# NVIDIA/nv-wavenet

Measured on AMD Instinct MI355X. Metric: samples/sec (all GPUs) in real time (every utterance >= 24 kHz) and max real-time batch @24kHz, R64/S256/A256 20L fp16, higher is better.
Workload: dtype f16; 1 GPU; C3: R=64 S=256 A=256 L=20 maxDilation=512 fp16, autoregressive generation at steady state (each step = samples 640..895 of every utterance: all dilated taps live, all rings wrapped; the steps re-run that sample range -- same launch, same memory traffic -- so from the second step on the rings hold the previous step's values: a timing workload, not one long utterance); batch_per_gpu=12288, global_batch=12288, parallelism=batch-sharded x1, final RCCL all_gather

## Files before the change

### nv_wavenet_amd/csrc/wn_experiments.hpp

```cpp
#pragma once

#ifndef WN_PFMAX
#define WN_PFMAX 12
#endif
#ifndef WN_PFMAX_FEAT
#define WN_PFMAX_FEAT 12
#endif
#ifndef WN_HEADREGS
#define WN_HEADREGS 128
#endif
#ifndef WN_HEADREGS2
#define WN_HEADREGS2 128
#endif
#ifndef WN_HEADREGS3
#define WN_HEADREGS3 0
#endif
#ifndef WN_COND_VALU
#define WN_COND_VALU 1
#endif
#ifndef WN_LDS_RING_MAXD
#define WN_LDS_RING_MAXD 512
#endif
#ifndef WN_SOFTMAX_2PASS
#define WN_SOFTMAX_2PASS 0
#endif
#ifndef WN_CHAIN_HOIST_FROM
#define WN_CHAIN_HOIST_FROM 4
#endif
#ifndef WN_WG4_FROM
#define WN_WG4_FROM 3
#endif
#ifndef WN_HEADREGS4
#define WN_HEADREGS4 0
#endif
#ifndef WN_ZS_B_REGS
#define WN_ZS_B_REGS 4096
#endif
#ifndef WN_ZA_B_REGS
#define WN_ZA_B_REGS 128
#endif
#ifndef WN_TAKE_G
#define WN_TAKE_G 1
#endif
#ifndef WN_REQ_AT
#define WN_REQ_AT 6
#endif
#ifndef WN_REQ_AT_FEAT
#define WN_REQ_AT_FEAT 6
#endif
#ifndef WN_UP_PHASES
#define WN_UP_PHASES(F16) 1
#endif
#ifndef WN_UP_COLS
#define WN_UP_COLS(F16) (WN_UP_PHASES(F16) > 1 ? 2 : 4)
#endif
#ifndef WN_UP_WAVES
#define WN_UP_WAVES(F16) (WN_UP_PHASES(F16) > 1 ? 8 : 4)
#endif
#ifndef WN_UP_ATTR
#define WN_UP_ATTR
#endif
#ifndef WN_W_AUX
#define WN_W_AUX 0
#endif
#ifndef WN_RING_LD_AUX
#define WN_RING_LD_AUX 2
#endif
#ifndef WN_RING_ST_AUX
#define WN_RING_ST_AUX 2
#endif
#ifndef WN_COND_AUX
#define WN_COND_AUX 2
#endif
#ifndef WN_RAW_AUX
#define WN_RAW_AUX 0
#endif
#ifndef WN_FEAT_AUX
#define WN_FEAT_AUX 0
#endif
```

### nv_wavenet_amd/csrc/wn_kernels.hpp

```cpp
#pragma once

#include <hip/hip_runtime.h>
#include <utility>
#include <stdint.h>

#include <type_traits>

#include "wn_experiments.hpp"

namespace wn {

#define WN_DEV __device__ __forceinline__

typedef _Float16 half8 __attribute__((ext_vector_type(8)));
typedef _Float16 half4 __attribute__((ext_vector_type(4)));
typedef float floatx4 __attribute__((ext_vector_type(4)));
typedef unsigned int uintx4 __attribute__((ext_vector_type(4)));
typedef unsigned int uintx2 __attribute__((ext_vector_type(2)));

template <bool F16> struct Prec;
template <> struct Prec<true> {
    using elem = _Float16;
    using frag = half8;
    using quad = half4;
    static constexpr int EPL = 8;
    static constexpr int TPF = 2;
};
template <> struct Prec<false> {
    using elem = float;
    using frag = floatx4;
    using quad = floatx4;
    static constexpr int EPL = 4;
    static constexpr int TPF = 1;
};

constexpr int kMaxLayers = 128;

constexpr int pick_pf(int fl, int pfmax) {
    int best = 1;
    for (int d = 1; d <= pfmax && d <= fl; d++)
        if (fl % d == 0) best = d;
    return best;
}
constexpr int align16(int x) { return (x + 15) & ~15; }

constexpr int kCondChannelsMax = 80;
template <bool F16> constexpr int feat_kfc() { return (kCondChannelsMax + 16 * Prec<F16>::TPF - 1) / (16 * Prec<F16>::TPF); }

template <bool F16, int R, int S, int A, int BT, int KFC = 0>
struct Cfg {
    using P = Prec<F16>;
    static constexpr int TPF = P::TPF, EPL = P::EPL;
    static constexpr int RT = R / 16, ST = S / 16, AT = A / 16;
    static constexpr int NW = RT >= 4 ? 4 : RT;
    static_assert(R % (16 * TPF) == 0 && S % (16 * TPF) == 0 && A % (16 * TPF) == 0, "R,S,A vs MFMA K step");
    static_assert(RT % NW == 0 && ST % NW == 0 && AT % NW == 0, "tiles must split evenly over the waves");
    static constexpr int THREADS = NW * 64;
    static constexpr int HTW = RT / NW, STW = ST / NW, ATW = AT / NW;
    static constexpr int KF_R = RT / TPF, KF_S = ST / TPF, KF_A = AT / TPF;
    static constexpr int FW_GATE = 2 * HTW * KF_R, FW_RES = HTW * KF_R, FW_SKIP = STW * KF_R, FW_COND = 2 * HTW * KFC;
    static constexpr int O_PREV = 0, O_CUR = FW_GATE, O_RES = 2 * FW_GATE, O_SKIP = O_RES + FW_RES, O_COND = O_SKIP + FW_SKIP;
    static constexpr int FLW = O_COND + FW_COND;
    __host__ __device__ static constexpr size_t streamPos(int l, int i, int L) {
        return i < O_CUR    ? (size_t)((l == 0 ? L : l) - 1) * FLW + FW_GATE + FW_COND + FW_RES + (i - O_PREV)
               : i < O_RES  ? (l == 0 ? (size_t)(i - O_CUR) : (size_t)l * FLW - FW_SKIP + (i - O_CUR))
               : i < O_SKIP ? (size_t)l * FLW + FW_GATE + FW_COND + (i - O_RES)
               : i < O_COND ? (l == L - 1 ? (size_t)L * FLW - FW_SKIP + (i - O_SKIP)
                                          : (size_t)(l + 1) * FLW - FW_SKIP + FW_GATE + (i - O_SKIP))
                            : (size_t)((l == 0 ? L : l) - 1) * FLW + FW_GATE + (i - O_COND);
    }
    static constexpr int P_CUR0 = FLW, P_CUR = FLW - FW_SKIP, P_SKIP = P_CUR + FW_GATE, P_COND = FLW + FW_GATE,
                         P_RES = P_COND + FW_COND, P_PREV = P_RES + FW_RES;
    static constexpr int FW_ZS = ATW * KF_S, FW_ZA = ATW * KF_A;
    static constexpr int FHW = FW_ZS + FW_ZA;
    static constexpr int PF = pick_pf(FLW, KFC > 0 ? WN_PFMAX_FEAT : WN_PFMAX);
    static_assert(FLW % PF == 0 && PF <= FW_ZS, "prefetch ring must divide the layer stream");
    static constexpr int HR = !F16 ? 0
                              : BT == 1 ? (FW_ZA * 4 <= WN_HEADREGS ? FW_ZA : 0)
                              : BT == 2 ? (FW_ZA * 4 <= WN_HEADREGS2 ? FW_ZA : 0)
                              : BT == 3 ? (FW_ZA * 4 <= WN_HEADREGS3 ? FW_ZA : 0)
                                        : (FW_ZA * 4 <= WN_HEADREGS4 ? FW_ZA : 0);
    static constexpr int HS = FHW - HR;
    static constexpr bool HEADRES = HS == 0;
    static constexpr int PAD1 = (PF - FW_ZS % PF) % PF, PAD2 = (PF - FW_ZA % PF) % PF;
    static constexpr int O_ZS = 0, O_ZA = FW_ZS + PAD1;
    static constexpr int FHWP = O_ZA + FW_ZA + PAD2;
    static constexpr int HSP = HS == 0 ? 0 : (HS == FW_ZS ? FW_ZS + PAD1 : FHWP);
    static_assert(HS == 0 || HS == FW_ZS || HS == FHW, "the streamed part of the head is nothing, zs, or all of it");
    __host__ __device__ static constexpr int headFrag(int q) { return q < FW_ZS ? q : q + PAD1; }
    static constexpr int FRAG_ELEMS = 64 * EPL;
    static constexpr int BIAS_L = 3 * R + S;
    static constexpr int COND_FR = 2 * HTW / TPF;
    static constexpr int LPU = 4 * NW;
    static constexpr int RPL = A / LPU;
    static_assert(RPL % 4 == 0, "A too small for the softmax lane split");
    static constexpr int XBUF = BT * KF_R * 1024;
    static constexpr int HBUF = XBUF;
    static constexpr int SKBUF = BT * KF_S * 1024;
    static constexpr int ZSBUF = BT * KF_A * 1024;
    static constexpr int LROW = A + 4;
    static constexpr int LGT = (BT >= 4 && WN_SOFTMAX_2PASS) ? 2 : BT;
    static_assert(BT % LGT == 0, "the softmax passes take whole groups of tiles");
    static constexpr int LGBUF = LGT * 16 * LROW * 4;
    static constexpr int YBUF = align16(BT * 16 * 4);
    static constexpr int XPBUF = XBUF;
    static constexpr int XPW = (KF_R + NW - 1) / NW;
    static constexpr bool ALIAS_LG = ZSBUF + LGBUF > 100 * 1024 || BT >= 3;
    static constexpr bool ZA_B_FROM_LDS = KF_A * BT * 4 > WN_ZA_B_REGS;
    static constexpr int HEADIMG = ALIAS_LG ? (ZSBUF > LGBUF ? ZSBUF : LGBUF) : ZSBUF + LGBUF;
    static constexpr bool OVERLAY = XBUF + HBUF + XPBUF <= (ALIAS_LG ? HEADIMG : LGBUF);
    static constexpr int OFF_SK = OVERLAY ? 0 : XBUF + HBUF, OFF_ZS = OFF_SK + SKBUF;
    static constexpr int OFF_LG = ALIAS_LG ? OFF_ZS : OFF_ZS + ZSBUF;
    static constexpr int OFF_Y = OFF_ZS + HEADIMG;
    static constexpr int OFF_X = OVERLAY ? OFF_LG : 0, OFF_H = OFF_X + XBUF, OFF_XP = OVERLAY ? OFF_H + HBUF : OFF_Y + YBUF;
    static constexpr int OFF_BIAS = OVERLAY ? OFF_Y + YBUF : OFF_XP + XPBUF;
    static constexpr int LDS_FIXED = XBUF + HBUF + SKBUF + HEADIMG + YBUF + XPBUF;
    static constexpr int BIAS_LN = 3 * R;
    __host__ __device__ static constexpr int biasFloats(int L, bool dump) { return (dump ? L * BIAS_L : L * BIAS_LN + S) + 2 * A; }
    __host__ __device__ static constexpr size_t ldsBytes(int L, int embTables, bool dump = true) {
        return (size_t)LDS_FIXED + (size_t)biasFloats(L, dump) * sizeof(float) + (size_t)embTables * A * R * sizeof(typename P::elem);
    }
    static constexpr int RING_SLOT = BT * KF_R * 1024;
    static constexpr int RING_INPLACE = OVERLAY ? 3 : 0;
    static_assert(XBUF == RING_SLOT && HBUF == RING_SLOT && XPBUF == RING_SLOT, "a vacated exchange image is one ring slot");
    static_assert(OFF_BIAS + RING_INPLACE * RING_SLOT == LDS_FIXED, "the in-place slots are what LDS_FIXED counts behind the tables");
    __host__ __device__ static constexpr int ringSlotOffset(int slot, int tailBase) { return tailBase + (slot - RING_INPLACE) * RING_SLOT; }
    __host__ __device__ static constexpr int ringTailSlots(int slots) { return slots > RING_INPLACE ? slots - RING_INPLACE : 0; }
    __host__ __device__ static constexpr int ldsRingSlots(int L, int maxDilation, int D) {
        int n = 0, d = 1;
        for (int l = 0; l < L; l++) {
            if (d <= D) n += d;
            d <<= 1;
            if (d > maxDilation) d = 1;
        }
        return n;
    }
    __host__ __device__ static size_t headOffsetFrags(int L) { return (size_t)L * FLW; }
    __host__ __device__ static size_t waveStreamFrags(int L) { return (size_t)L * FLW + FHWP; }
};

struct Dil {
    int d, off, lds;
};
WN_DEV Dil dil_first() { return Dil{1, 0, 0}; }
WN_DEV Dil dil_next(Dil s, int maxDilation, bool wrapToFirst, int ldsD = 0) {
    Dil n;
    n.off = s.off + s.d;
    n.lds = s.lds + (s.d <= ldsD ? s.d : 0);
    n.d = s.d << 1;
    if (n.d > maxDilation) n.d = 1;
    if (wrapToFirst) n = dil_first();
    return n;
}

struct Params {
    const void* wblob;
    const float* bias;
    const void* embPrev;
    const void* embCur;
    const void* cond;
    const void* condRaw;
    int condRawKind;
    const void* feat;
    const unsigned* gate;
    const float* sel;
    void* ring;
    int maxDilation;
    int* yInPrev;
    int* yInCur;
    int* yOut;
    float* xtOut;
    float* skipOut;
// ... 140 lines not shown
    if constexpr (PIN) return __builtin_bit_cast(FRAG, agpr_pin(__builtin_bit_cast(floatx4, f)));
    else return f;
}

template <bool F16, int PF, bool PIN = F16> struct WStream {
    typename Prec<F16>::frag buf[PF];
};

template <bool F16, int PF, int WRAP, bool PIN>
WN_DEV typename Prec<F16>::frag take(WStream<F16, PF, PIN>& ws, int idx, const char* base, const char* wrapBase,
                                     unsigned laneOff, int rtWrapAt = 0x7fffffff, long rtWrapDelta = 0) {
    using frag = typename Prec<F16>::frag;
    frag a = agpr_operand<F16 && PIN>(ws.buf[idx % PF]);
    int nidx = idx + PF;
    const char* src = (WRAP > 0 && nidx >= WRAP) ? wrapBase + (size_t)(nidx - WRAP) * 1024 : base + (size_t)nidx * 1024;
    if (nidx >= rtWrapAt) src += rtWrapDelta;
    ws.buf[idx % PF] = *(const frag*)(src + laneOff);
    __builtin_amdgcn_sched_barrier(0);
    return a;
}

template <bool F16, int PF, int WRAP, int BT, int MT, int KF, bool PIN>
WN_DEV void gemm(WStream<F16, PF, PIN>& ws, int pos0, const char* cur, const char* next, unsigned laneOff,
                 floatx4 (&acc)[BT][MT], const typename Prec<F16>::frag (&b)[BT][KF], int rtWrapAt = 0x7fffffff,
                 long rtWrapDelta = 0) {
    constexpr int G = MT >= 4 ? 4 : MT;
#pragma unroll
    for (int mg = 0; mg < MT / G; mg++) {
#pragma unroll
        for (int kf = 0; kf < KF; kf++) {
#pragma unroll
            for (int mi = 0; mi < G; mi++) {
                const int mt = mg * G + mi;
                auto a = take<F16, PF, WRAP>(ws, pos0 + (mg * KF + kf) * G + mi, cur, next, laneOff, rtWrapAt, rtWrapDelta);
#pragma unroll
                for (int bt = 0; bt < BT; bt++) acc[bt][mt] = mma(a, b[bt][kf], acc[bt][mt]);
            }
        }
    }
}

template <bool F16, int PF, int WRAP, int BT, int MT, int KF, bool PIN>
WN_DEV void gemm_ldsb(WStream<F16, PF, PIN>& ws, int pos0, const char* cur, const char* next, unsigned laneOff,
                      floatx4 (&acc)[BT][MT], const char* bimg, int lane) {
    using frag = typename Prec<F16>::frag;
    constexpr int G = MT >= 4 ? 4 : MT;
#pragma unroll
    for (int mg = 0; mg < MT / G; mg++) {
#pragma unroll
        for (int kf = 0; kf < KF; kf++) {
            frag b[BT];
#pragma unroll
            for (int bt = 0; bt < BT; bt++) b[bt] = *(const frag*)(bimg + (((bt * KF + kf) * 64 + lane) << 4));
#pragma unroll
            for (int mi = 0; mi < G; mi++) {
                const int mt = mg * G + mi;
                auto a = take<F16, PF, WRAP>(ws, pos0 + (mg * KF + kf) * G + mi, cur, next, laneOff);
#pragma unroll
                for (int bt = 0; bt < BT; bt++) acc[bt][mt] = mma(a, b[bt], acc[bt][mt]);
            }
        }
    }
}

typedef __amdgpu_buffer_rsrc_t rsrc_t;
__host__ __device__ constexpr int take_g(int g, int pf) {
    int t = g < WN_TAKE_G ? g : WN_TAKE_G;
    t = t < pf ? t : pf;
    while (g % t) t--;
    return t;
}
WN_DEV rsrc_t make_rsrc(const void* p) { return __builtin_amdgcn_make_buffer_rsrc((void*)p, 0, -1, 0x00020000); }
template <typename FRAG, int AUX = 0> WN_DEV FRAG buf_load(rsrc_t rs, unsigned voff, unsigned soff) {
    return __builtin_bit_cast(FRAG, __builtin_amdgcn_raw_buffer_load_b128(rs, voff, soff, AUX));
}
template <typename FRAG, int AUX = 0> WN_DEV void buf_store(rsrc_t rs, unsigned voff, unsigned soff, FRAG v) {
    __builtin_amdgcn_raw_buffer_store_b128(__builtin_bit_cast(uintx4, v), rs, voff, soff, AUX);
}
template <bool F16, int PF, bool PIN, int G>
WN_DEV void take_group(WStream<F16, PF, PIN>& ws, int idx, typename Prec<F16>::frag (&a)[G]) {
#pragma unroll
    for (int i = G - 1; i >= 0; i--) a[i] = agpr_operand<F16 && PIN>(ws.buf[(idx + i) % PF]);
}
template <bool F16, int PF, int WRAP, bool PIN, int G>
WN_DEV void refill_group(WStream<F16, PF, PIN>& ws, rsrc_t rs, int idx, int basePos, int wrapPos, unsigned laneOff) {
    using frag = typename Prec<F16>::frag;
#pragma unroll
    for (int i = 0; i < G; i++) {
        const int nidx = idx + i + PF;
        const bool wr = WRAP > 0 && nidx >= WRAP;
        const int rel = wr ? nidx - WRAP : nidx;
        const int pos = (wr ? wrapPos : basePos) + (rel & ~3);
        ws.buf[(idx + i) % PF] = buf_load<frag, WN_W_AUX>(rs, laneOff + (unsigned)(rel & 3) * 1024u, (unsigned)pos * 1024u);
    }
    __builtin_amdgcn_sched_barrier(0);
}
template <bool F16, int PF, int WRAP, int BT, int MT, int KF, bool PIN>
WN_DEV void gemm_b(WStream<F16, PF, PIN>& ws, rsrc_t rs, int pos0, int basePos, int wrapPos, unsigned laneOff,
                   floatx4 (&acc)[BT][MT], const typename Prec<F16>::frag (&b)[BT][KF]) {
    constexpr int G = MT >= 4 ? 4 : MT;
#pragma unroll
    for (int mg = 0; mg < MT / G; mg++) {
#pragma unroll
        for (int kf = 0; kf < KF; kf++) {
            constexpr int TG = take_g(G, PF);
#pragma unroll
            for (int m0 = 0; m0 < G; m0 += TG) {
                typename Prec<F16>::frag a[TG];
                const int idx = pos0 + (mg * KF + kf) * G + m0;
                take_group<F16, PF, PIN, TG>(ws, idx, a);
                constexpr bool EARLY = PF > TG;
                if (EARLY && !(mg == 0 && kf == 0 && m0 == 0)) refill_group<F16, PF, WRAP, PIN, TG>(ws, rs, idx - TG, basePos, wrapPos, laneOff);
#pragma unroll
                for (int mi = 0; mi < TG; mi++)
#pragma unroll
                    for (int bt = 0; bt < BT; bt++)
                        acc[bt][mg * G + m0 + mi] = mma(a[mi], b[bt][kf], acc[bt][mg * G + m0 + mi]);
                if (!EARLY || (mg == MT / G - 1 && kf == KF - 1 && m0 + TG >= G)) refill_group<F16, PF, WRAP, PIN, TG>(ws, rs, idx, basePos, wrapPos, laneOff);
            }
        }
    }
}
template <bool F16, int PF, int WRAP, int BT, int MT, int KF, bool PIN>
WN_DEV void gemm_ldsb_b(WStream<F16, PF, PIN>& ws, rsrc_t rs, int pos0, int basePos, int wrapPos, unsigned laneOff,
                        floatx4 (&acc)[BT][MT], const char* bimg, int lane) {
    using frag = typename Prec<F16>::frag;
    constexpr int G = MT >= 4 ? 4 : MT;
#pragma unroll
    for (int mg = 0; mg < MT / G; mg++) {
#pragma unroll
        for (int kf = 0; kf < KF; kf++) {
            frag b[BT];
#pragma unroll
            for (int bt = 0; bt < BT; bt++) b[bt] = *(const frag*)(bimg + (((bt * KF + kf) * 64 + lane) << 4));
            constexpr int TG = take_g(G, PF);
#pragma unroll
            for (int m0 = 0; m0 < G; m0 += TG) {
                frag a[TG];
                take_group<F16, PF, PIN, TG>(ws, pos0 + (mg * KF + kf) * G + m0, a);
#pragma unroll
                for (int mi = 0; mi < TG; mi++)
#pragma unroll
                    for (int bt = 0; bt < BT; bt++) acc[bt][mg * G + m0 + mi] = mma(a[mi], b[bt], acc[bt][mg * G + m0 + mi]);
                refill_group<F16, PF, WRAP, PIN, TG>(ws, rs, pos0 + (mg * KF + kf) * G + m0, basePos, wrapPos, laneOff);
            }
        }
    }
}
template <bool F16, int PF, int WRAP, bool PIN, int N>
WN_DEV void skip_frags(WStream<F16, PF, PIN>& ws, rsrc_t rs, int idx, int basePos, int wrapPos, unsigned laneOff) {
    if constexpr (N > 0) {
        typename Prec<F16>::frag a[N];
        take_group<F16, PF, PIN, N>(ws, idx, a);
        refill_group<F16, PF, WRAP, PIN, N>(ws, rs, idx, basePos, wrapPos, laneOff);
    }
}

template <bool F16, int BT, int MT, int KF>
WN_DEV void gemm_direct(const char* src, unsigned laneOff, floatx4 (&acc)[BT][MT], const typename Prec<F16>::frag (&b)[BT][KF]) {
    using frag = typename Prec<F16>::frag;
    constexpr int G = MT >= 4 ? 4 : MT;
#pragma unroll
    for (int mg = 0; mg < MT / G; mg++)
#pragma unroll
        for (int kf = 0; kf < KF; kf++)
#pragma unroll
            for (int mi = 0; mi < G; mi++) {
                const frag a = *(const frag*)(src + (size_t)((mg * KF + kf) * G + mi) * 1024 + laneOff);
#pragma unroll
                for (int bt = 0; bt < BT; bt++) acc[bt][mg * G + mi] = mma(a, b[bt][kf], acc[bt][mg * G + mi]);
            }
}

template <bool F16, int BT, int MT, int KF, int NFR>
WN_DEV void gemm_res(const typename Prec<F16>::frag (&wres)[NFR], int pos0, floatx4 (&acc)[BT][MT],
                     const typename Prec<F16>::frag (&b)[BT][KF]) {
    constexpr int G = MT >= 4 ? 4 : MT;
#pragma unroll
    for (int mg = 0; mg < MT / G; mg++)
#pragma unroll
        for (int kf = 0; kf < KF; kf++)
#pragma unroll
            for (int mi = 0; mi < G; mi++)
#pragma unroll
                for (int bt = 0; bt < BT; bt++)
                    acc[bt][mg * G + mi] = mma(agpr_operand<F16>(wres[pos0 + (mg * KF + kf) * G + mi]), b[bt][kf], acc[bt][mg * G + mi]);
}

template <int CTRL> WN_DEV float dpp_f(float v) {
    return __int_as_float(__builtin_amdgcn_update_dpp(0, __float_as_int(v), CTRL, 0xf, 0xf, false));
}
template <int CTRL> WN_DEV int dpp_i(int v) { return __builtin_amdgcn_update_dpp(0, v, CTRL, 0xf, 0xf, false); }
constexpr int DPP_XOR1 = 0xB1, DPP_XOR2 = 0x4E;
constexpr int DPP_HALF_MIRROR = 0x141, DPP_MIRROR = 0x140;
template <int LPU, typename F> WN_DEV float group_reduce_f(float v, F op) {
    static_assert(LPU == 4 || LPU == 8 || LPU == 16, "softmax lanes per utterance");
    v = op(v, dpp_f<DPP_XOR1>(v));
    v = op(v, dpp_f<DPP_XOR2>(v));
    if (LPU >= 8) v = op(v, dpp_f<DPP_HALF_MIRROR>(v));
    if (LPU >= 16) v = op(v, dpp_f<DPP_MIRROR>(v));
    return v;
}
template <int LPU> WN_DEV int group_min_i(int v) {
    int o = dpp_i<DPP_XOR1>(v); v = o < v ? o : v;
    o = dpp_i<DPP_XOR2>(v); v = o < v ? o : v;
    if (LPU >= 8) { o = dpp_i<DPP_HALF_MIRROR>(v); v = o < v ? o : v; }
    if (LPU >= 16) { o = dpp_i<DPP_MIRROR>(v); v = o < v ? o : v; }
    return v;
}

template <int A, int LPU, int RPL>
WN_DEV int softmax_pick(const float* lrow, int sq, int lane, float sel, float (&e)[RPL], float& total) {
    (void)lane;
#pragma unroll
    for (int i = 0; i < RPL / 4; i++) {
        floatx4 v = *(const floatx4*)(lrow + i * 4);
#pragma unroll
        for (int r = 0; r < 4; r++) e[i * 4 + r] = v[r];
    }
    float m = e[0];
#pragma unroll
    for (int i = 1; i < RPL; i++) m = __builtin_fmaxf(m, e[i]);
    m = group_reduce_f<LPU>(m, [](float a, float b) { return __builtin_fmaxf(a, b); });
    float lsum = 0.f;
    {
        constexpr float kLog2e = 1.44269504088896340736f;
        const float mneg = -m * kLog2e;
#pragma unroll
        for (int i = 0; i < RPL; i++) {
            e[i] = __builtin_amdgcn_exp2f(__builtin_fmaf(e[i], kLog2e, mneg));
            lsum += e[i];
        }
    }
    float incl = lsum;
    {
        float up = dpp_f<0x111>(incl);
        if (sq >= 1) incl += up;
        up = dpp_f<0x112>(incl);
// ... 333 lines not shown
    for (int tt = 0; tt < P::TPF; tt++)
#pragma unroll
        for (int e = 0; e < P::EPL; e++)
            selA[tt][e] = (elem)(((e >> 2) == tt && g * 4 + (e & 3) == j) ? 1.0f : 0.0f);
    floatx4 acc[BT][2 * HTW];
    {
        frag xp[BT][KF_R];
#pragma unroll
        for (int bt = 0; bt < BT; bt++) {
            lds_get_frags<F16, KF_R>(tap_image(p.dil[0], p.initSample) + bt * KF_R * 1024, lane, xp[bt]);
#pragma unroll
            for (int i = 0; i < HTW; i++) {
                acc[bt][2 * i] = *(const floatx4*)(biasLds + (w + NW * i) * 16 + g * 4);
                acc[bt][2 * i + 1] = *(const floatx4*)(biasLds + (w + NW * i + RT) * 16 + g * 4);
            }
        }
        if constexpr (FEAT) {
            load_feat(p.initSample, cfNext);
#pragma unroll
            for (int bt = 0; bt < BT; bt++)
#pragma unroll
                for (int k = 0; k < KFC; k++) cfCur[bt][k] = agpr_operand<F16>(cfNext[bt][k]);
            gemm_direct<F16, BT, 2 * HTW, KFC>(wbase + C::streamPos(0, C::O_COND, L) * 1024, laneOff, acc, cfCur);
            load_feat(p.initSample + 1, cfNext);
#pragma unroll
            for (int bt = 0; bt < BT; bt++)
#pragma unroll
                for (int k = 0; k < KFC; k++) asm volatile("" ::"v"(cfNext[bt][k]));
        } else {
#pragma unroll
            for (int bt = 0; bt < BT; bt++)
#pragma unroll
                for (int k = 0; k < C::COND_FR; k++) cond_add<F16>(&acc[bt][k * P::TPF], cond_frag<F16, RAW>(cdA[bt], k), selA);
        }
        gemm_direct<F16, BT, 2 * HTW, KF_R>(wbase + C::streamPos(0, C::O_PREV, L) * 1024, laneOff, acc, xp);
    }
    const int tEnd = p.initSample + p.count;
    for (int t = p.initSample; t < tEnd; t++) {
        const bool dumpNow = DUMP && p.dump && (t == tEnd - 1);

        float selv[BT];
        if (!p.useRng) {
#pragma unroll
            for (int bt = 0; bt < BT; bt++) {
                int sb = (tile0 + bt) * 16 + su;
                sb = sb < p.batch ? sb : p.batch - 1;
                selv[bt] = p.sel[(size_t)t * p.maxBatch + sb];
            }
        }

        WN_TMARK(11)
        floatx4 x[BT][HTW];
#pragma unroll
        for (int bt = 0; bt < BT; bt++) {
#pragma unroll
            for (int i = 0; i < HTW; i++) {
                const int tile = w + NW * i;
                floatx4 ec = quad_to_f32(*(const quad*)(embCur + (size_t)yCur[bt] * R + tile * 16 + g * 4));
                floatx4 v = ep[bt][i] + ec;
                if (p.tanhEmbed) {
#pragma unroll
                    for (int r = 0; r < 4; r++) v[r] = tanh_t<F16>(v[r]);
                }
                x[bt][i] = v;
                lds_put_tile<F16>(xbuf + bt * KF_R * 1024, tile, lane, v);
            }
#pragma unroll
            for (int i = 0; i < HTW; i++)
                ep[bt][i] = quad_to_f32(*(const quad*)(embPrev + (size_t)yCur[bt] * R + (w + NW * i) * 16 + g * 4));
        }
        wg_barrier();
        WN_TMARK(0)

        floatx4 skip[BT][STW];
#pragma unroll
        for (int bt = 0; bt < BT; bt++)
#pragma unroll
            for (int i = 0; i < STW; i++) skip[bt][i] = floatx4{0.f, 0.f, 0.f, 0.f};

        frag hb[BT][KF_R];
        frag xb[BT][KF_R];
#pragma unroll
        for (int bt = 0; bt < BT; bt++) lds_get_frags<F16, KF_R>(xbuf + bt * KF_R * 1024, lane, xb[bt]);
        auto layer = [&](auto withSkip, const int l, const Dil dl, const Dil dN, const Dil dl2, frag (&xpC)[BT][XPW],
                         frag (&cdC)[BT][CR], const frag (&xpN)[BT][XPW], const frag (&cdN)[BT][CR]) {
            constexpr bool SKIP = decltype(withSkip)::value;
            constexpr int PB = SKIP ? 0 : FLW;
            const int wl = SKIP ? (l - 1) * FLW : 0;
            const float* bl = biasLds + l * BLS;
            const int lN = l + 1 < L ? l + 1 : 0;
            const float* blN = biasLds + lN * BLS;
            const int d = dl.d;

            WN_TMARK(1)
            gemm_b<F16, PF, 0, BT, 2 * HTW, KF_R>(ws, rsW, SKIP ? C::P_CUR : C::P_CUR0 - PB, wl, 0, laneOff, acc, xb);
            const bool ringInLds = d <= ldsD;
            frag xkeep[BT][XPW];
            if (!ringInLds) {
                const unsigned rp = (unsigned)(dl.off + (t & (d - 1))) * (unsigned)(KF_R * 1024);
#pragma unroll
                for (int k = 0; k < KF_R; k++)
                    if (k % NW == w) {
#pragma unroll
                        for (int bt = 0; bt < BT; bt++)
                            buf_store<frag, WN_RING_ST_AUX>(rsRing, laneOff + (unsigned)(k & 3) * 1024u,
                                               rp + (unsigned)bt * ringTileB + (unsigned)(k & ~3) * 1024u, xb[bt][k]);
                    }
            } else {
#pragma unroll
                for (int k = 0; k < KF_R; k++)
                    if (k % NW == w) {
#pragma unroll
                        for (int bt = 0; bt < BT; bt++) xkeep[bt][k / NW] = xb[bt][k];
                    }
            }
            if constexpr (!SKIP) prefetch(t, l + 2, dl2, xpC, cdC);
            __builtin_amdgcn_sched_barrier(0);
            WN_TMARK(2)

            floatx4 accN[FEAT ? BT : 1][2 * HTW];
            if constexpr (FEAT) {
#pragma unroll
                for (int bt = 0; bt < BT; bt++)
#pragma unroll
                    for (int i = 0; i < HTW; i++) {
                        accN[bt][2 * i] = *(const floatx4*)(blN + (w + NW * i) * 16 + g * 4);
                        accN[bt][2 * i + 1] = *(const floatx4*)(blN + (w + NW * i + RT) * 16 + g * 4);
                    }
            }
            if constexpr (FEAT) {
                constexpr int NS = BT * HTW * 2 * 5;
                constexpr int NFS = SKIP ? STW * KF_R : 0, NFC = C::FW_COND;
                constexpr int NM = (NFS + NFC) * BT;
                constexpr int G0S = STW >= 4 ? 4 : STW, G0C = 2 * HTW >= 4 ? 4 : 2 * HTW;
                constexpr bool EARLY = PF > 1;
                floatx2 ea, eb, ra, rb, hp;
                floatx4 hv;
                auto stage = [&](auto SI) {
                    constexpr int s = decltype(SI)::value, pr = s / 5, st = s % 5;
                    constexpr int bt = pr / (2 * HTW), i = (pr / 2) % HTW, r = (pr & 1) * 2;
                    gate_stage<F16, st>(acc[bt][2 * i][r], acc[bt][2 * i][r + 1], acc[bt][2 * i + 1][r], acc[bt][2 * i + 1][r + 1],
                                        ea, eb, ra, rb, hp);
                    if constexpr (st == 4) {
                        hv[r] = hp[0];
                        hv[r + 1] = hp[1];
                        if constexpr (r == 2) lds_put_tile<F16>(hbuf + bt * KF_R * 1024, w + NW * i, lane, hv);
                    }
                    __builtin_amdgcn_sched_barrier(0);
                };
                static_for<NFS + NFC>([&](auto FI) {
                    constexpr int fi = decltype(FI)::value;
                    constexpr bool isSkip = fi < NFS;
                    constexpr int q = isSkip ? fi : fi - NFS, G0 = isSkip ? G0S : G0C, KFq = isSkip ? KF_R : KFC;
                    constexpr int kf = (q / G0) % KFq, mt = (q / (G0 * KFq)) * G0 + q % G0;
                    constexpr int pos = isSkip ? C::P_SKIP + q : C::P_COND - PB + q;
                    constexpr int posPrev = (fi - 1 < NFS) ? C::P_SKIP + fi - 1 : C::P_COND - PB + fi - 1 - NFS;
                    frag a[1];
                    take_group<F16, PF, ws_pin, 1>(ws, pos, a);
                    if constexpr (EARLY && fi > 0) refill_group<F16, PF, 0, ws_pin, 1>(ws, rsW, posPrev, wl, 0, laneOff);
                    static_for<BT>([&](auto BI) {
                        constexpr int bt = decltype(BI)::value, m = fi * BT + bt;
                        if constexpr (isSkip) skip[bt][mt] = mma(a[0], hb[bt][kf], skip[bt][mt]);
                        else accN[bt][mt] = mma(a[0], cfCur[bt][kf], accN[bt][mt]);
                        __builtin_amdgcn_sched_barrier(0);
                        static_for_range<m * NS / NM, (m + 1) * NS / NM>(stage);
                    });
                    if constexpr (!EARLY || fi == NFS + NFC - 1) refill_group<F16, PF, 0, ws_pin, 1>(ws, rsW, pos, wl, 0, laneOff);
                    if constexpr (SKIP && fi == (NFS + NFC) * WN_REQ_AT_FEAT / 8) {
                        prefetch(t, l + 2, dl2, xpC, cdC);
                        __builtin_amdgcn_sched_barrier(0);
                    }
                });
                if (l == L - 2) {
                    asm volatile("");
#pragma unroll
                    for (int bt = 0; bt < BT; bt++)
#pragma unroll
                        for (int k = 0; k < KFC; k++) cfCur[bt][k] = agpr_operand<F16>(cfNext[bt][k]);
                }
                if constexpr (SKIP) {
                    if (dumpNow) {
                        const float* bp = biasLds + (l - 1) * C::BIAS_L + 3 * R;
#pragma unroll
                        for (int bt = 0; bt < BT; bt++) {
                            if (!uvalid[bt]) continue;
#pragma unroll
                            for (int i = 0; i < STW; i++)
                                *(floatx4*)(p.skipOut + ((size_t)(l - 1) * p.maxBatch + ub[bt]) * S + (w + NW * i) * 16 + g * 4) =
                                    skip[bt][i] + *(const floatx4*)(bp + (w + NW * i) * 16 + g * 4);
                        }
                    }
                }
            } else {
                constexpr int NS = BT * HTW * 2 * 5;
                constexpr int NM = SKIP ? STW * KF_R * BT : 0;
                floatx2 ea, eb, ra, rb, hp;
                floatx4 hv;
                auto stage = [&](auto SI) {
                    constexpr int s = decltype(SI)::value, pr = s / 5, st = s % 5;
                    constexpr int bt = pr / (2 * HTW), i = (pr / 2) % HTW, r = (pr & 1) * 2;
                    gate_stage<F16, st>(acc[bt][2 * i][r], acc[bt][2 * i][r + 1], acc[bt][2 * i + 1][r], acc[bt][2 * i + 1][r + 1],
                                        ea, eb, ra, rb, hp);
                    if constexpr (st == 4) {
                        hv[r] = hp[0];
                        hv[r + 1] = hp[1];
                        if constexpr (r == 2) lds_put_tile<F16>(hbuf + bt * KF_R * 1024, w + NW * i, lane, hv);
                    }
                    __builtin_amdgcn_sched_barrier(0);
                };
                if constexpr (SKIP) {
                    constexpr int G0 = STW >= 4 ? 4 : STW, G = take_g(G0, PF);
                    static_for<STW * KF_R / G>([&](auto GI) {
                        constexpr int gi = decltype(GI)::value, q = gi * G;
                        constexpr int kf = (q / G0) % KF_R, mg = q / (G0 * KF_R), mi0 = q % G0;
                        frag a[G];
                        take_group<F16, PF, ws_pin, G>(ws, C::P_SKIP + gi * G, a);
                        constexpr bool EARLY = PF > G;
                        if constexpr (EARLY && gi > 0) refill_group<F16, PF, 0, ws_pin, G>(ws, rsW, C::P_SKIP + (gi - 1) * G, wl, 0, laneOff);
                        static_for<G * BT>([&](auto MI) {
                            constexpr int mi = decltype(MI)::value / BT, bt = decltype(MI)::value % BT;
                            constexpr int mt = mg * G0 + mi0 + mi, m = (q + mi) * BT + bt;
                            skip[bt][mt] = mma(a[mi], hb[bt][kf], skip[bt][mt]);
                            __builtin_amdgcn_sched_barrier(0);
                            static_for_range<m * NS / NM, (m + 1) * NS / NM>(stage);
                        });
                        if constexpr (!EARLY || gi == STW * KF_R / G - 1) refill_group<F16, PF, 0, ws_pin, G>(ws, rsW, C::P_SKIP + gi * G, wl, 0, laneOff);
                        if constexpr (gi == (STW * KF_R / G) * WN_REQ_AT / 8) {
                            prefetch(t, l + 2, dl2, xpC, cdC);
                            __builtin_amdgcn_sched_barrier(0);
                        }
                    });
                    if (dumpNow) {
                        const float* bp = biasLds + (l - 1) * C::BIAS_L + 3 * R;
#pragma unroll
                        for (int bt = 0; bt < BT; bt++) {
                            if (!uvalid[bt]) continue;
#pragma unroll
                            for (int i = 0; i < STW; i++)
                                *(floatx4*)(p.skipOut + ((size_t)(l - 1) * p.maxBatch + ub[bt]) * S + (w + NW * i) * 16 + g * 4) =
                                    skip[bt][i] + *(const floatx4*)(bp + (w + NW * i) * 16 + g * 4);
                        }
                    }
                } else {
                    static_for<NS>(stage);
                }
            }
            WN_TMARK(3)
            wg_barrier();
            WN_TMARK(4)
#pragma unroll
            for (int bt = 0; bt < BT; bt++) lds_get_frags<F16, KF_R>(hbuf + bt * KF_R * 1024, lane, hb[bt]);
            if (ringInLds) {
                char* const sl = ringLds + (size_t)(dl.lds + (t & (d - 1))) * C::RING_SLOT;
#pragma unroll
                for (int i = 0; i < XPW; i++) {
                    const int k = w + NW * i;
                    if (k < KF_R) {
#pragma unroll
                        for (int bt = 0; bt < BT; bt++) *(frag*)(sl + ((bt * KF_R + k) * 64 + lane) * 16) = xkeep[bt][i];
                    }
                }
            }

            floatx4 xa[BT][HTW];
#pragma unroll
            for (int bt = 0; bt < BT; bt++)
#pragma unroll
                for (int i = 0; i < HTW; i++)
                    xa[bt][i] = *(const floatx4*)(bl + 2 * R + (w + NW * i) * 16 + g * 4) + x[bt][i];
#pragma unroll
            for (int bt = 0; bt < BT; bt++)
#pragma unroll
                for (int i = 0; i < HTW; i++) {
                    if constexpr (FEAT) {
                        acc[bt][2 * i] = accN[bt][2 * i];
                        acc[bt][2 * i + 1] = accN[bt][2 * i + 1];
                    } else {
                        acc[bt][2 * i] = *(const floatx4*)(blN + (w + NW * i) * 16 + g * 4);
                        acc[bt][2 * i + 1] = *(const floatx4*)(blN + (w + NW * i + RT) * 16 + g * 4);
                    }
                }

            gemm_b<F16, PF, 0, BT, HTW, KF_R>(ws, rsW, C::P_RES - PB, wl, 0, laneOff, xa, hb);
#pragma unroll
            for (int bt = 0; bt < BT; bt++)
#pragma unroll
                for (int i = 0; i < HTW; i++) {
                    x[bt][i] = xa[bt][i];
                    lds_put_tile<F16>(xbuf + bt * KF_R * 1024, w + NW * i, lane, xa[bt][i]);
                }
            publish_xp(xpN, dN);
            __builtin_amdgcn_sched_barrier(0);
            WN_TMARK(5)
            if constexpr (FEAT) {
            } else {
#pragma unroll
                for (int bt = 0; bt < BT; bt++)
#pragma unroll
                    for (int k = 0; k < C::COND_FR; k++) cond_add<F16>(&acc[bt][k * P::TPF], cond_frag<F16, RAW>(cdN[bt], k), selA);
            }
            if (dumpNow) {
#pragma unroll
                for (int bt = 0; bt < BT; bt++) {
                    if (!uvalid[bt]) continue;
#pragma unroll
                    for (int i = 0; i < HTW; i++)
                        *(floatx4*)(p.xtOut + ((size_t)l * p.maxBatch + ub[bt]) * R + (w + NW * i) * 16 + g * 4) = x[bt][i];
                }
            }
            __builtin_amdgcn_sched_barrier(0);
            WN_TMARK(6)
            wg_barrier();
            WN_TMARK(7)
            frag xp[BT][KF_R];
            const char* const tapImg = tap_image(dN, l + 1 < L ? t : t + 1);
#pragma unroll
            for (int bt = 0; bt < BT; bt++) lds_get_frags<F16, KF_R>(tapImg + bt * KF_R * 1024, lane, xp[bt]);
#pragma unroll
            for (int bt = 0; bt < BT; bt++) lds_get_frags<F16, KF_R>(xbuf + bt * KF_R * 1024, lane, xb[bt]);
            __builtin_amdgcn_sched_barrier(0);
            gemm_b<F16, PF, 0, BT, 2 * HTW, KF_R>(ws, rsW, C::P_PREV - PB, wl, 0, laneOff, acc, xp);
        };
        {
            Dil da = dil_first(), db = dil_next(da, p.maxDilation, L == 1, ldsD), dc = dil_next(db, p.maxDilation, L == 2, ldsD);
            auto adv = [&](int l) { da = db; db = dc; dc = dil_next(dc, p.maxDilation, l + 3 == L, ldsD); };
            layer(std::false_type{}, 0, da, db, dc, xpA, cdA, xpB, cdB);
            adv(0);
            int l = 1;
            for (; l + 1 < L; l += 2) {
                layer(std::true_type{}, l, da, db, dc, xpB, cdB, xpA, cdA);
                adv(l);
                layer(std::true_type{}, l + 1, da, db, dc, xpA, cdA, xpB, cdB);
                adv(l + 1);
            }
            if (l < L) layer(std::true_type{}, l, da, db, dc, xpB, cdB, xpA, cdA);
            if (L & 1) {
#pragma unroll
                for (int bt = 0; bt < BT; bt++) {
#pragma unroll
                    for (int i = 0; i < XPW; i++) {
                        const frag tmp = xpA[bt][i];
                        xpA[bt][i] = xpB[bt][i];
                        xpB[bt][i] = tmp;
                    }
#pragma unroll
                    for (int k = 0; k < CR; k++) {
                        const frag tmp = cdA[bt][k];
                        cdA[bt][k] = cdB[bt][k];
                        cdB[bt][k] = tmp;
                    }
                }
            }
        }
        gemm_b<F16, PF, 0, BT, STW, KF_R>(ws, rsW, C::P_CUR, (L - 1) * FLW, 0, laneOff, skip, hb);

#pragma unroll
        for (int bt = 0; bt < BT; bt++)
#pragma unroll
            for (int i = 0; i < STW; i++) {
                floatx4 v = skip[bt][i] + *(const floatx4*)(skipBiasSum + (w + NW * i) * 16 + g * 4);
#pragma unroll
                for (int r = 0; r < 4; r++) v[r] = __builtin_fmaxf(v[r], 0.f);
                lds_put_tile<F16>(skbuf + bt * KF_S * 1024, w + NW * i, lane, v);
                if (dumpNow && uvalid[bt])
                    *(floatx4*)(p.skipOut + ((size_t)(L - 1) * p.maxBatch + ub[bt]) * S + (w + NW * i) * 16 + g * 4) = v;
            }
        wg_barrier();
        floatx4 zs[BT][ATW];
        if constexpr (HS != 0 && KF_S * BT * 4 > WN_ZS_B_REGS) {
#pragma unroll
            for (int bt = 0; bt < BT; bt++)
#pragma unroll
                for (int i = 0; i < ATW; i++) zs[bt][i] = *(const floatx4*)(headBias + (w + NW * i) * 16 + g * 4);
            gemm_ldsb_b<F16, PF, C::HSP, BT, ATW, KF_S>(ws, rsW, C::O_ZS, L * FLW, 0, laneOff, zs, skbuf, lane);
            skip_frags<F16, PF, C::HSP, ws_pin, C::PAD1>(ws, rsW, C::FW_ZS, L * FLW, 0, laneOff);
        } else {
            frag sb[BT][KF_S];
#pragma unroll
            for (int bt = 0; bt < BT; bt++) {
                lds_get_frags<F16, KF_S>(skbuf + bt * KF_S * 1024, lane, sb[bt]);
#pragma unroll
                for (int i = 0; i < ATW; i++) zs[bt][i] = *(const floatx4*)(headBias + (w + NW * i) * 16 + g * 4);
            }
            if constexpr (HS == 0) gemm_res<F16, BT, ATW, KF_S>(hw, 0, zs, sb);
            else {
                gemm_b<F16, PF, C::HSP, BT, ATW, KF_S>(ws, rsW, C::O_ZS, L * FLW, 0, laneOff, zs, sb);
                skip_frags<F16, PF, C::HSP, ws_pin, C::PAD1>(ws, rsW, C::FW_ZS, L * FLW, 0, laneOff);
            }
        }
#pragma unroll
        for (int bt = 0; bt < BT; bt++)
#pragma unroll
            for (int i = 0; i < ATW; i++) {
#pragma unroll
                for (int r = 0; r < 4; r++) zs[bt][i][r] = __builtin_fmaxf(zs[bt][i][r], 0.f);
                lds_put_tile<F16>(zsbuf + bt * KF_A * 1024, w + NW * i, lane, zs[bt][i]);
                if (dumpNow && uvalid[bt])
                    *(floatx4*)(p.zs + (size_t)ub[bt] * A + (w + NW * i) * 16 + g * 4) = zs[bt][i];
            }
        wg_barrier();
        floatx4 za[BT][ATW];
        {
#pragma unroll
            for (int bt = 0; bt < BT; bt++)
#pragma unroll
                for (int i = 0; i < ATW; i++)
                    za[bt][i] = *(const floatx4*)(headBias + A + (w + NW * i) * 16 + g * 4);
            auto draw_selectors = [&]() {
                if (!p.useRng) return;
                if constexpr (C::LPU == 16 && BT > 1) {
                    const int q = sq < BT ? sq : 0;
                    int sb = (tile0 + q) * 16 + su;
                    sb = sb < p.batch ? sb : p.batch - 1;
                    const float mine = philox_selector(p.rngKey0, p.rngKey1, (unsigned)t, (unsigned)sb);
                    selv[0] = dpp_f<0x150>(mine);
                    if constexpr (BT > 1) selv[1] = dpp_f<0x151>(mine);
                    if constexpr (BT > 2) selv[2] = dpp_f<0x152>(mine);
                    if constexpr (BT > 3) selv[3] = dpp_f<0x153>(mine);
                } else {
#pragma unroll
                    for (int bt = 0; bt < BT; bt++) {
                        int sb = (tile0 + bt) * 16 + su;
                        sb = sb < p.batch ? sb : p.batch - 1;
                        selv[bt] = philox_selector(p.rngKey0, p.rngKey1, (unsigned)t, (unsigned)sb);
                    }
                }
            };
            if constexpr (C::ZA_B_FROM_LDS) {
                static_assert(HR == 0, "the LDS-streamed head is for the large, non-resident heads");
                draw_selectors();
                gemm_ldsb_b<F16, PF, C::HSP, BT, ATW, KF_A>(ws, rsW, C::O_ZA, L * FLW, 0, laneOff, za, zsbuf, lane);
            } else {
                frag zb[BT][KF_A];
#pragma unroll
                for (int bt = 0; bt < BT; bt++) lds_get_frags<F16, KF_A>(zsbuf + bt * KF_A * 1024, lane, zb[bt]);
                draw_selectors();
                if constexpr (HR >= C::FW_ZA) gemm_res<F16, BT, ATW, KF_A>(hw, C::FW_ZS - HS, za, zb);
                else gemm_b<F16, PF, C::HSP, BT, ATW, KF_A>(ws, rsW, C::O_ZA, L * FLW, 0, laneOff, za, zb);
            }
        }
        if constexpr (C::ALIAS_LG) wg_barrier();
        constexpr int LGT = C::LGT;
        auto put_logits = [&](auto PASS) {
            constexpr int pass = decltype(PASS)::value;
#pragma unroll
            for (int bl = 0; bl < LGT; bl++)
#pragma unroll
                for (int i = 0; i < ATW; i++) {
                    const int bt = pass * LGT + bl;
                    *(floatx4*)(lgbuf + (bl * 16 + j) * C::LROW + (w + NW * i) * 16 + g * 4) = za[bt][i];
                    if (dumpNow && uvalid[bt])
                        *(floatx4*)(p.za + (size_t)ub[bt] * A + (w + NW * i) * 16 + g * 4) = za[bt][i];
                }
        };
        put_logits(std::integral_constant<int, 0>{});
        WN_TMARK(8)
        if constexpr (HS == FHW) {
            skip_frags<F16, PF, C::HSP, ws_pin, C::PAD2>(ws, rsW, C::O_ZA + C::FW_ZA, L * FLW, 0, laneOff);
        }
        if constexpr (FEAT) load_feat(t + 2, cfNext);
        wg_barrier();
        WN_TMARK(9)

        static_for<BT / LGT>([&](auto PASS) {
            constexpr int pass = decltype(PASS)::value;
            if constexpr (pass > 0) {
                wg_barrier();
                put_logits(PASS);
                wg_barrier();
            }
#pragma unroll
            for (int bl = 0; bl < LGT; bl++) {
                const int bt = pass * LGT + bl;
                float e[C::RPL];
                float total;
                const float* lrow = lgbuf + (bl * 16 + su) * C::LROW + sq * C::RPL;
                const int pick = softmax_pick<A, C::LPU, C::RPL>(lrow, sq, lane, selv[bt], e, total);
                const int sb = (tile0 + bt) * 16 + su;
                if (sq == 0) {
                    ybuf[bt * 16 + su] = pick;
                    if (sb < p.batch) p.yOut[(size_t)sb * p.numSamples + t] = pick;
                }
                if (dumpNow && sb < p.batch) {
                    const float inv = 1.0f / total;
#pragma unroll
                    for (int i = 0; i < C::RPL / 4; i++)
                        *(floatx4*)(p.p + (size_t)sb * A + sq * C::RPL + i * 4) =
                            floatx4{e[i * 4] * inv, e[i * 4 + 1] * inv, e[i * 4 + 2] * inv, e[i * 4 + 3] * inv};
                }
            }
        });
        wg_barrier();
#pragma unroll
        for (int bt = 0; bt < BT; bt++) {
            yPrev[bt] = yCur[bt];
            yCur[bt] = ybuf[bt * 16 + j];
        }
        WN_TMARK(10)
    }
#ifdef WN_TIMING
    if (tid == 0 && blockIdx.x == 0)
        for (int i = 0; i < 12; i++) p.p[i] = (float)tacc[i];
#endif

    ring_lds_copy(std::false_type{});
    if (w == 0 && g == 0) {
#pragma unroll
        for (int bt = 0; bt < BT; bt++)
            if (uvalid[bt]) {
                p.yInPrev[ub[bt]] = yPrev[bt];
                p.yInCur[ub[bt]] = yCur[bt];
            }
    }
    if (p.clk != nullptr && blockIdx.x == 0 && tid == 0) {
        p.clk[2] = __builtin_amdgcn_s_memtime();
        p.clk[3] = __builtin_amdgcn_s_memrealtime();
    }
}

static __global__ void mulaw_pcm_kernel(const int* __restrict__ yOut, short* __restrict__ pcm,
                                        const short* __restrict__ table, int batch, int numSamples, int first,
                                        int count) {
    const size_t n = (size_t)batch * count;
    for (size_t i = blockIdx.x * (size_t)blockDim.x + threadIdx.x; i < n; i += (size_t)gridDim.x * blockDim.x) {
        const size_t at = (i / count) * numSamples + first + (i % count);
        pcm[at] = table[yOut[at]];
    }
}


template <bool F16>
WN_DEV void pack_weight_elem(typename Prec<F16>::elem* __restrict__ dst, const float* __restrict__ src, int M, int K,
                             int NW, size_t waveStride, int gateRT, size_t idx) {
    constexpr int EPL = Prec<F16>::EPL, TPF = Prec<F16>::TPF;
    const int KF = K / (16 * TPF);
    const int tilesPerWave = M / 16 / NW;
    const size_t perWave = (size_t)tilesPerWave * KF * 64 * EPL;
    const int w = idx / perWave;
    size_t r = idx % perWave;
    const int e = r % EPL; r /= EPL;
    const int lane = r % 64; r /= 64;
// ... 297 lines not shown
```

Before: 329.2 million samples/s.

## Skip last layer's unused residual GEMM and head pad-fragment weight loads

The final layer's residual GEMM is skipped when not dumping, since its output is never consumed; its weight fragments are advanced through the prefetch ring with refills only. Prefetch refills that would land on padding fragments in the head stream are dropped, and skip_frags now only issues the trailing refills instead of taking and refilling every fragment. An experimental knob (off by default) can store short-dilation ring entries with different cache bits. The risk is stale prefetch-ring slots if the skip logic misaligns the stream positions.

Result: no change. 330.6 million samples/s (median of 6 runs) (+0.4%).

```diff
diff --git a/nv_wavenet_amd/csrc/wn_experiments.hpp b/nv_wavenet_amd/csrc/wn_experiments.hpp
--- a/nv_wavenet_amd/csrc/wn_experiments.hpp
+++ b/nv_wavenet_amd/csrc/wn_experiments.hpp
@@ -69,6 +69,9 @@
 #ifndef WN_RING_ST_AUX
 #define WN_RING_ST_AUX 2
 #endif
+#ifndef WN_EXP_RING_L2_D
+#define WN_EXP_RING_L2_D 0
+#endif
 #ifndef WN_COND_AUX
 #define WN_COND_AUX 2
 #endif
diff --git a/nv_wavenet_amd/csrc/wn_kernels.hpp b/nv_wavenet_amd/csrc/wn_kernels.hpp
--- a/nv_wavenet_amd/csrc/wn_kernels.hpp
+++ b/nv_wavenet_amd/csrc/wn_kernels.hpp
@@ -88,6 +88,9 @@
     static constexpr int HSP = HS == 0 ? 0 : (HS == FW_ZS ? FW_ZS + PAD1 : FHWP);
     static_assert(HS == 0 || HS == FW_ZS || HS == FHW, "the streamed part of the head is nothing, zs, or all of it");
     __host__ __device__ static constexpr int headFrag(int q) { return q < FW_ZS ? q : q + PAD1; }
+    __host__ __device__ static constexpr bool headPad(int off) {
+        return off >= 0 && off < HSP && ((off >= FW_ZS && off < O_ZA) || off >= O_ZA + FW_ZA);
+    }
     static constexpr int FRAG_ELEMS = 64 * EPL;
     static constexpr int BIAS_L = 3 * R + S;
     static constexpr int COND_FR = 2 * HTW / TPF;
@@ -394,7 +397,10 @@
 #pragma unroll
     for (int i = G - 1; i >= 0; i--) a[i] = agpr_operand<F16 && PIN>(ws.buf[(idx + i) % PF]);
 }
-template <bool F16, int PF, int WRAP, bool PIN, int G>
+struct NoHeadPads {
+    __host__ __device__ static constexpr bool headPad(int) { return false; }
+};
+template <bool F16, int PF, int WRAP, bool PIN, int G, class HP = NoHeadPads>
 WN_DEV void refill_group(WStream<F16, PF, PIN>& ws, rsrc_t rs, int idx, int basePos, int wrapPos, unsigned laneOff) {
     using frag = typename Prec<F16>::frag;
 #pragma unroll
@@ -402,12 +408,13 @@
         const int nidx = idx + i + PF;
         const bool wr = WRAP > 0 && nidx >= WRAP;
         const int rel = wr ? nidx - WRAP : nidx;
+        if (WRAP > 0 && !wr && HP::headPad(nidx)) continue;
         const int pos = (wr ? wrapPos : basePos) + (rel & ~3);
         ws.buf[(idx + i) % PF] = buf_load<frag, WN_W_AUX>(rs, laneOff + (unsigned)(rel & 3) * 1024u, (unsigned)pos * 1024u);
     }
     __builtin_amdgcn_sched_barrier(0);
 }
-template <bool F16, int PF, int WRAP, int BT, int MT, int KF, bool PIN>
+template <bool F16, int PF, int WRAP, int BT, int MT, int KF, class HP = NoHeadPads, bool PIN>
 WN_DEV void gemm_b(WStream<F16, PF, PIN>& ws, rsrc_t rs, int pos0, int basePos, int wrapPos, unsigned laneOff,
                    floatx4 (&acc)[BT][MT], const typename Prec<F16>::frag (&b)[BT][KF]) {
     constexpr int G = MT >= 4 ? 4 : MT;
@@ -422,18 +429,18 @@
                 const int idx = pos0 + (mg * KF + kf) * G + m0;
                 take_group<F16, PF, PIN, TG>(ws, idx, a);
                 constexpr bool EARLY = PF > TG;
-                if (EARLY && !(mg == 0 && kf == 0 && m0 == 0)) refill_group<F16, PF, WRAP, PIN, TG>(ws, rs, idx - TG, basePos, wrapPos, laneOff);
+                if (EARLY && !(mg == 0 && kf == 0 && m0 == 0)) refill_group<F16, PF, WRAP, PIN, TG, HP>(ws, rs, idx - TG, basePos, wrapPos, laneOff);
 #pragma unroll
                 for (int mi = 0; mi < TG; mi++)
 #pragma unroll
                     for (int bt = 0; bt < BT; bt++)
                         acc[bt][mg * G + m0 + mi] = mma(a[mi], b[bt][kf], acc[bt][mg * G + m0 + mi]);
-                if (!EARLY || (mg == MT / G - 1 && kf == KF - 1 && m0 + TG >= G)) refill_group<F16, PF, WRAP, PIN, TG>(ws, rs, idx, basePos, wrapPos, laneOff);
-            }
-        }
-    }
-}
-template <bool F16, int PF, int WRAP, int BT, int MT, int KF, bool PIN>
+                if (!EARLY || (mg == MT / G - 1 && kf == KF - 1 && m0 + TG >= G)) refill_group<F16, PF, WRAP, PIN, TG, HP>(ws, rs, idx, basePos, wrapPos, laneOff);
+            }
+        }
+    }
+}
+template <bool F16, int PF, int WRAP, int BT, int MT, int KF, class HP = NoHeadPads, bool PIN>
 WN_DEV void gemm_ldsb_b(WStream<F16, PF, PIN>& ws, rsrc_t rs, int pos0, int basePos, int wrapPos, unsigned laneOff,
                         floatx4 (&acc)[BT][MT], const char* bimg, int lane) {
     using frag = typename Prec<F16>::frag;
@@ -454,18 +461,15 @@
                 for (int mi = 0; mi < TG; mi++)
 #pragma unroll
                     for (int bt = 0; bt < BT; bt++) acc[bt][mg * G + m0 + mi] = mma(a[mi], b[bt], acc[bt][mg * G + m0 + mi]);
-                refill_group<F16, PF, WRAP, PIN, TG>(ws, rs, pos0 + (mg * KF + kf) * G + m0, basePos, wrapPos, laneOff);
-            }
-        }
-    }
-}
-template <bool F16, int PF, int WRAP, bool PIN, int N>
+                refill_group<F16, PF, WRAP, PIN, TG, HP>(ws, rs, pos0 + (mg * KF + kf) * G + m0, basePos, wrapPos, laneOff);
+            }
+        }
+    }
+}
+template <bool F16, int PF, int WRAP, bool PIN, int N, class HP = NoHeadPads>
 WN_DEV void skip_frags(WStream<F16, PF, PIN>& ws, rsrc_t rs, int idx, int basePos, int wrapPos, unsigned laneOff) {
-    if constexpr (N > 0) {
-        typename Prec<F16>::frag a[N];
-        take_group<F16, PF, PIN, N>(ws, idx, a);
-        refill_group<F16, PF, WRAP, PIN, N>(ws, rs, idx, basePos, wrapPos, laneOff);
-    }
+    constexpr int M = N < PF ? N : PF;
+    if constexpr (M > 0) refill_group<F16, PF, WRAP, PIN, M, HP>(ws, rs, idx + N - M, basePos, wrapPos, laneOff);
 }
 
 template <bool F16, int BT, int MT, int KF>
@@ -965,9 +969,11 @@
         frag xb[BT][KF_R];
 #pragma unroll
         for (int bt = 0; bt < BT; bt++) lds_get_frags<F16, KF_R>(xbuf + bt * KF_R * 1024, lane, xb[bt]);
-        auto layer = [&](auto withSkip, const int l, const Dil dl, const Dil dN, const Dil dl2, frag (&xpC)[BT][XPW],
+        auto layer = [&](auto withSkip, auto lastNoRes, const int l, const Dil dl, const Dil dN, const Dil dl2, frag (&xpC)[BT][XPW],
                          frag (&cdC)[BT][CR], const frag (&xpN)[BT][XPW], const frag (&cdN)[BT][CR]) {
             constexpr bool SKIP = decltype(withSkip)::value;
+            constexpr bool NORES = decltype(lastNoRes)::value;
+            static_assert(!(NORES && DUMP), "a dumping kernel writes the last layer's residual to xtOut");
             constexpr int PB = SKIP ? 0 : FLW;
             const int wl = SKIP ? (l - 1) * FLW : 0;
             const float* bl = biasLds + l * BLS;
@@ -985,9 +991,14 @@
                 for (int k = 0; k < KF_R; k++)
                     if (k % NW == w) {
 #pragma unroll
-                        for (int bt = 0; bt < BT; bt++)
-                            buf_store<frag, WN_RING_ST_AUX>(rsRing, laneOff + (unsigned)(k & 3) * 1024u,
-                                               rp + (unsigned)bt * ringTileB + (unsigned)(k & ~3) * 1024u, xb[bt][k]);
+                        for (int bt = 0; bt < BT; bt++) {
+                            if (WN_EXP_RING_L2_D > 0 && d <= WN_EXP_RING_L2_D)
+                                buf_store<frag, 0>(rsRing, laneOff + (unsigned)(k & 3) * 1024u,
+                                                   rp + (unsigned)bt * ringTileB + (unsigned)(k & ~3) * 1024u, xb[bt][k]);
+                            else
+                                buf_store<frag, WN_RING_ST_AUX>(rsRing, laneOff + (unsigned)(k & 3) * 1024u,
+                                                   rp + (unsigned)bt * ringTileB + (unsigned)(k & ~3) * 1024u, xb[bt][k]);
+                        }
                     }
             } else {
 #pragma unroll
@@ -1146,11 +1157,13 @@
             }
 
             floatx4 xa[BT][HTW];
-#pragma unroll
-            for (int bt = 0; bt < BT; bt++)
-#pragma unroll
-                for (int i = 0; i < HTW; i++)
-                    xa[bt][i] = *(const floatx4*)(bl + 2 * R + (w + NW * i) * 16 + g * 4) + x[bt][i];
+            if constexpr (!NORES) {
+#pragma unroll
+                for (int bt = 0; bt < BT; bt++)
+#pragma unroll
+                    for (int i = 0; i < HTW; i++)
+                        xa[bt][i] = *(const floatx4*)(bl + 2 * R + (w + NW * i) * 16 + g * 4) + x[bt][i];
+            }
 #pragma unroll
             for (int bt = 0; bt < BT; bt++)
 #pragma unroll
@@ -1164,14 +1177,18 @@
                     }
                 }
 
-            gemm_b<F16, PF, 0, BT, HTW, KF_R>(ws, rsW, C::P_RES - PB, wl, 0, laneOff, xa, hb);
-#pragma unroll
-            for (int bt = 0; bt < BT; bt++)
-#pragma unroll
-                for (int i = 0; i < HTW; i++) {
-                    x[bt][i] = xa[bt][i];
-                    lds_put_tile<F16>(xbuf + bt * KF_R * 1024, w + NW * i, lane, xa[bt][i]);
-                }
+            if constexpr (NORES) {
+                skip_frags<F16, PF, 0, ws_pin, HTW * KF_R>(ws, rsW, C::P_RES - PB, wl, 0, laneOff);
+            } else {
+                gemm_b<F16, PF, 0, BT, HTW, KF_R>(ws, rsW, C::P_RES - PB, wl, 0, laneOff, xa, hb);
+#pragma unroll
+                for (int bt = 0; bt < BT; bt++)
+#pragma unroll
+                    for (int i = 0; i < HTW; i++) {
+                        x[bt][i] = xa[bt][i];
+                        lds_put_tile<F16>(xbuf + bt * KF_R * 1024, w + NW * i, lane, xa[bt][i]);
+                    }
+            }
             publish_xp(xpN, dN);
             __builtin_amdgcn_sched_barrier(0);
             WN_TMARK(5)
@@ -1199,24 +1216,26 @@
             const char* const tapImg = tap_image(dN, l + 1 < L ? t : t + 1);
 #pragma unroll
             for (int bt = 0; bt < BT; bt++) lds_get_frags<F16, KF_R>(tapImg + bt * KF_R * 1024, lane, xp[bt]);
-#pragma unroll
-            for (int bt = 0; bt < BT; bt++) lds_get_frags<F16, KF_R>(xbuf + bt * KF_R * 1024, lane, xb[bt]);
+            if constexpr (!NORES) {
+#pragma unroll
+                for (int bt = 0; bt < BT; bt++) lds_get_frags<F16, KF_R>(xbuf + bt * KF_R * 1024, lane, xb[bt]);
+            }
             __builtin_amdgcn_sched_barrier(0);
             gemm_b<F16, PF, 0, BT, 2 * HTW, KF_R>(ws, rsW, C::P_PREV - PB, wl, 0, laneOff, acc, xp);
         };
         {
             Dil da = dil_first(), db = dil_next(da, p.maxDilation, L == 1, ldsD), dc = dil_next(db, p.maxDilation, L == 2, ldsD);
             auto adv = [&](int l) { da = db; db = dc; dc = dil_next(dc, p.maxDilation, l + 3 == L, ldsD); };
-            layer(std::false_type{}, 0, da, db, dc, xpA, cdA, xpB, cdB);
+            layer(std::false_type{}, std::false_type{}, 0, da, db, dc, xpA, cdA, xpB, cdB);
             adv(0);
             int l = 1;
             for (; l + 1 < L; l += 2) {
-                layer(std::true_type{}, l, da, db, dc, xpB, cdB, xpA, cdA);
+                layer(std::true_type{}, std::false_type{}, l, da, db, dc, xpB, cdB, xpA, cdA);
                 adv(l);
-                layer(std::true_type{}, l + 1, da, db, dc, xpA, cdA, xpB, cdB);
+                layer(std::true_type{}, std::false_type{}, l + 1, da, db, dc, xpA, cdA, xpB, cdB);
                 adv(l + 1);
             }
-            if (l < L) layer(std::true_type{}, l, da, db, dc, xpB, cdB, xpA, cdA);
+            if (l < L) layer(std::true_type{}, std::bool_constant<!DUMP>{}, l, da, db, dc, xpB, cdB, xpA, cdA);
             if (L & 1) {
 #pragma unroll
                 for (int bt = 0; bt < BT; bt++) {
@@ -1255,8 +1274,8 @@
             for (int bt = 0; bt < BT; bt++)
 #pragma unroll
                 for (int i = 0; i < ATW; i++) zs[bt][i] = *(const floatx4*)(headBias + (w + NW * i) * 16 + g * 4);
-            gemm_ldsb_b<F16, PF, C::HSP, BT, ATW, KF_S>(ws, rsW, C::O_ZS, L * FLW, 0, laneOff, zs, skbuf, lane);
-            skip_frags<F16, PF, C::HSP, ws_pin, C::PAD1>(ws, rsW, C::FW_ZS, L * FLW, 0, laneOff);
+            gemm_ldsb_b<F16, PF, C::HSP, BT, ATW, KF_S, C>(ws, rsW, C::O_ZS, L * FLW, 0, laneOff, zs, skbuf, lane);
+            skip_frags<F16, PF, C::HSP, ws_pin, C::PAD1, C>(ws, rsW, C::FW_ZS, L * FLW, 0, laneOff);
         } else {
             frag sb[BT][KF_S];
 #pragma unroll
@@ -1267,8 +1286,8 @@
             }
             if constexpr (HS == 0) gemm_res<F16, BT, ATW, KF_S>(hw, 0, zs, sb);
             else {
-                gemm_b<F16, PF, C::HSP, BT, ATW, KF_S>(ws, rsW, C::O_ZS, L * FLW, 0, laneOff, zs, sb);
-                skip_frags<F16, PF, C::HSP, ws_pin, C::PAD1>(ws, rsW, C::FW_ZS, L * FLW, 0, laneOff);
+                gemm_b<F16, PF, C::HSP, BT, ATW, KF_S, C>(ws, rsW, C::O_ZS, L * FLW, 0, laneOff, zs, sb);
+                skip_frags<F16, PF, C::HSP, ws_pin, C::PAD1, C>(ws, rsW, C::FW_ZS, L * FLW, 0, laneOff);
             }
         }
 #pragma unroll
@@ -1312,14 +1331,14 @@
             if constexpr (C::ZA_B_FROM_LDS) {
                 static_assert(HR == 0, "the LDS-streamed head is for the large, non-resident heads");
                 draw_selectors();
-                gemm_ldsb_b<F16, PF, C::HSP, BT, ATW, KF_A>(ws, rsW, C::O_ZA, L * FLW, 0, laneOff, za, zsbuf, lane);
+                gemm_ldsb_b<F16, PF, C::HSP, BT, ATW, KF_A, C>(ws, rsW, C::O_ZA, L * FLW, 0, laneOff, za, zsbuf, lane);
             } else {
                 frag zb[BT][KF_A];
 #pragma unroll
                 for (int bt = 0; bt < BT; bt++) lds_get_frags<F16, KF_A>(zsbuf + bt * KF_A * 1024, lane, zb[bt]);
                 draw_selectors();
                 if constexpr (HR >= C::FW_ZA) gemm_res<F16, BT, ATW, KF_A>(hw, C::FW_ZS - HS, za, zb);
-                else gemm_b<F16, PF, C::HSP, BT, ATW, KF_A>(ws, rsW, C::O_ZA, L * FLW, 0, laneOff, za, zb);
+                else gemm_b<F16, PF, C::HSP, BT, ATW, KF_A, C>(ws, rsW, C::O_ZA, L * FLW, 0, laneOff, za, zb);
             }
         }
         if constexpr (C::ALIAS_LG) wg_barrier();
@@ -1339,7 +1358,7 @@
         put_logits(std::integral_constant<int, 0>{});
         WN_TMARK(8)
         if constexpr (HS == FHW) {
-            skip_frags<F16, PF, C::HSP, ws_pin, C::PAD2>(ws, rsW, C::O_ZA + C::FW_ZA, L * FLW, 0, laneOff);
+            skip_frags<F16, PF, C::HSP, ws_pin, C::PAD2, C>(ws, rsW, C::O_ZA + C::FW_ZA, L * FLW, 0, laneOff);
         }
         if constexpr (FEAT) load_feat(t + 2, cfNext);
         wg_barrier();
```
